# saltoricristiano/lidog

Measured on AMD Instinct MI355X. Metric: LiDAR scans/sec, MinkUNet34+BEV training step @120k pts, higher is better.
Workload: dtype f32

## Files before the change

### include/lidog_amd.h

```cpp
#ifndef LIDOG_AMD_H
#define LIDOG_AMD_H

#include <stdint.h>

#ifdef __cplusplus
extern "C" {
#endif

const char *lidog_last_error(void);
int lidog_abi_version(void);


int64_t lidog_hash_capacity(int64_t n);

int lidog_coords_insert(const int32_t *coords, int64_t n, uint64_t *keys, int32_t *vals, int64_t cap,
                        int32_t *first_row, int64_t *n_unique_dev, int32_t *err_flag, void *stream);
int lidog_coords_insert_info(const int32_t *coords, int64_t n, uint64_t *keys, int32_t *vals, int64_t cap,
                             int32_t *first_row, int64_t *info, int32_t *err_flag, void *stream);

int lidog_coords_compact(const int32_t *first_row, int64_t n, const uint64_t *keys, int32_t *vals, int64_t cap,
                         const int32_t *coords, int32_t *unique_rows, int32_t *inverse, int32_t *scan_ws,
                         void *stream);

int lidog_coords_stride(const int32_t *coords_in, int64_t n_in, int32_t new_stride, uint64_t *keys,
                        int32_t *vals, int64_t cap, int32_t *parent2child, int32_t *coords_out,
                        int64_t *n_out_dev, int32_t *ws, int32_t *err_flag, void *stream);

int64_t lidog_bitmap_words(int32_t nx, int32_t ny, int32_t nz, int32_t nb, int64_t max_bytes);
int lidog_bitmap_set(const int32_t *coords, int64_t n, int32_t x0, int32_t y0, int32_t z0, int32_t nx, int32_t ny,
                     int32_t nz, int32_t stride, int32_t nb, uint32_t *bits, int32_t *err_flag, void *stream);
int lidog_kernel_map_bits(const int32_t *coords_out, int64_t n_out, const uint64_t *in_keys, const int32_t *in_vals,
                          int64_t in_cap, const int32_t *offsets_host, int32_t K, const uint32_t *bits, int32_t x0,
                          int32_t y0, int32_t z0, int32_t nx, int32_t ny, int32_t nz, int32_t stride, int32_t nb,
                          int32_t *nbr, void *stream);
int lidog_kernel_map_subset(const int32_t *nbr_big, int64_t n, int32_t K_big, const int32_t *sel_host, int32_t K,
                            int32_t *nbr, void *stream);

int lidog_kernel_map(const int32_t *coords_out, int64_t n_out, const uint64_t *in_keys, const int32_t *in_vals,
                     int64_t in_cap, const int32_t *offsets_host, int32_t K, int32_t *nbr, void *stream);

int lidog_kernel_map_pairs(const int32_t *nbr, int64_t n_out, int64_t n_in, int32_t K, int64_t *k_off_dev,
                           int32_t *pair_in, int32_t *pair_out, int32_t *pos_out, int32_t *pos_in, int32_t *ws,
                           void *stream);
int lidog_kernel_map_rows(const int32_t *pos, int64_t n, int32_t K, int32_t mark_k, int32_t *row_ptr,
                          int32_t *row_list, int32_t *ws, void *stream);


int lidog_sconv_gemm(const float *A, const int32_t *gather, const float *B, const float *bias,
                     const int32_t *tile_k, const int32_t *tile_row0, const int32_t *tile_rows, int32_t n_tiles,
                     int32_t Cin, int32_t Cout, float *T, const int32_t *scatter, int64_t a_rows, void *stream);
int32_t lidog_sconv_gemm_units(int32_t multi, int32_t slots);
int lidog_sconv_gemm_addend(const float *A, const int32_t *gather, const float *B, const int32_t *tile_k,
                            const int32_t *tile_row0, const int32_t *tile_rows, int32_t n_tiles, int32_t Cin,
                            int32_t Cout, const float *addend, float *T, const int32_t *scatter, void *stream);

int lidog_sconv_reduce(const float *T, const int32_t *pos, int64_t n, int32_t K, int32_t C, const float *bias,
                       const float *addend ,
                       float *out, void *stream);

int64_t lidog_sconv_reduce_stats_ws(int64_t n, int32_t C);
int lidog_sconv_reduce_stats(const float *T, const int32_t *pos, int64_t n, int32_t K, int32_t C, const float *bias,
                             float *out, double *sums, double *partial_ws, double count, float eps, float momentum,
                             float *mean, float *invstd, float *running_mean, float *running_var, void *stream);
int lidog_sconv_reduce_rows(const float *T, const int32_t *row_ptr, const int32_t *row_list, int64_t n, int32_t C,
                            const float *bias, const float *addend, float *out, void *stream);
int lidog_sconv_reduce_rows_stats(const float *T, const int32_t *row_ptr, const int32_t *row_list, int64_t n,
                                  int32_t C, const float *bias, float *out, double *sums, double *partial_ws,
                                  double count, float eps, float momentum, float *mean, float *invstd,
// ... 287 lines not shown
```

### lidog_amd/_lib.py

```python
import ctypes
import os

import torch

_HERE = os.path.dirname(os.path.abspath(__file__))
SO_PATH = os.environ.get("LIDOG_SO") or os.path.join(_HERE, "_C", "liblidog_amd.so")

_i32, _i64, _p, _f, _d = ctypes.c_int32, ctypes.c_int64, ctypes.c_void_p, ctypes.c_float, ctypes.c_double

SIGNATURES = {
    "lidog_abi_version": [],
    "lidog_hash_capacity": [_i64],
    "lidog_coords_insert": [_p, _i64, _p, _p, _i64, _p, _p, _p, _p],
    "lidog_coords_insert_info": [_p, _i64, _p, _p, _i64, _p, _p, _p, _p],
    "lidog_coords_compact": [_p, _i64, _p, _p, _i64, _p, _p, _p, _p, _p],
    "lidog_coords_stride": [_p, _i64, _i32, _p, _p, _i64, _p, _p, _p, _p, _p, _p],
    "lidog_kernel_map": [_p, _i64, _p, _p, _i64, _p, _i32, _p, _p],
    "lidog_bitmap_words": [_i32, _i32, _i32, _i32, _i64],
    "lidog_bitmap_set": [_p, _i64, _i32, _i32, _i32, _i32, _i32, _i32, _i32, _i32, _p, _p, _p],
    "lidog_kernel_map_bits": [_p, _i64, _p, _p, _i64, _p, _i32, _p, _i32, _i32, _i32, _i32, _i32, _i32, _i32, _i32, _p, _p],
    "lidog_kernel_map_pairs": [_p, _i64, _i64, _i32, _p, _p, _p, _p, _p, _p, _p],
    "lidog_sconv_gemm_units": [_i32, _i32],
    "lidog_sconv_gemm": [_p, _p, _p, _p, _p, _p, _p, _i32, _i32, _i32, _p, _p, _i64, _p],
    "lidog_sconv_gemm_addend": [_p, _p, _p, _p, _p, _p, _i32, _i32, _i32, _p, _p, _p, _p],
    "lidog_sconv_reduce": [_p, _p, _i64, _i32, _i32, _p, _p, _p, _p],
    "lidog_sconv_reduce_stats_ws": [_i64, _i32],
    "lidog_sconv_reduce_stats": [_p, _p, _i64, _i32, _i32, _p, _p, _p, _p, _d, _f, _f, _p, _p, _p, _p, _p],
    "lidog_kernel_map_rows": [_p, _i64, _i32, _i32, _p, _p, _p, _p],
    "lidog_sconv_reduce_rows": [_p, _p, _p, _i64, _i32, _p, _p, _p, _p],
    "lidog_sconv_reduce_rows_bn": [_p, _p, _p, _i64, _i32, _p, _p, _p, _p, _p, _p, _i32, _p, _p],
    "lidog_sconv_reduce_rows_stats": [_p, _p, _p, _i64, _i32, _p, _p, _p, _p, _d, _f, _f, _p, _p, _p, _p, _p],
    "lidog_sconv_reduce_rows_bwdstats": [_p, _p, _p, _i64, _i32, _p, _p, _p, _p, _p, _p, _p, _p, _p, _p, _p, _d, _p, _p, _p],
    "lidog_bn_bwd_reduce_blocks": [_i64, _i32],
    "lidog_stats_max_blocks": [],
    "lidog_sconv_cin1": [_p, _p, _p, _p, _i64, _i32, _i32, _p, _p],
    "lidog_kernel_map_subset": [_p, _i64, _i32, _p, _i32, _p, _p],
    "lidog_kernel_map_sorted_ws": [_i64],
    "lidog_kernel_map_sorted": [_p, _i64, _i32, _p, _p, _p, _p, _p, _i64, _p],
    "lidog_sconv_os": [_p, _p, _i64, _i32, _p, _p, _p, _p, _i32, _p, _p, _i32, _i32, _p, _p],
    "lidog_sconv_os_stats_ws": [_i64, _i32],
    "lidog_sconv_os_bn": [_p, _p, _i64, _i32, _p, _p, _p, _p, _p, _i32, _i32, _p, _p, _p, _p, _p, _i32, _p, _p],
    "lidog_sconv_os_stats": [_p, _p, _i64, _i32, _p, _p, _p, _p, _p, _i32, _i32, _p, _p, _p, _d, _f, _f, _p, _p, _p, _p, _p],
    "lidog_sconv_wgrad": [_p, _p, _p, _p, _p, _i32, _p, _i32, _i32, _i32, _p, _p, _p],
    "lidog_sconv_gemm_in_bn": [_p, _p, _p, _p, _p, _p, _p, _i32, _i32, _i32, _p, _p, _p, _p, _p, _p, _i32, _i64, _p],
# ... 190 lines not shown
```

### lidog_amd/csrc/coords.hip

```cpp
#include <limits.h>
#include <stdarg.h>

#include "common.h"

static thread_local char g_err[512] = "";
void lidog_set_error(const char *fmt, ...) {
    va_list ap;
    va_start(ap, fmt);
    vsnprintf(g_err, sizeof(g_err), fmt, ap);
    va_end(ap);
}
extern "C" const char *lidog_last_error(void) { return g_err; }
extern "C" int lidog_abi_version(void) { return 8; }

extern "C" int64_t lidog_hash_capacity(int64_t n) {
    int64_t cap = 1024;
    while (cap < 2 * n) cap <<= 1;
    return cap;
}

__device__ __forceinline__ int block_excl_scan_256(int v, int *total) {
    __shared__ int wsum[4];
    const int lane = threadIdx.x & 63, w = threadIdx.x >> 6;
    int x = v;
// ... 51 lines not shown
    int v[4], s = 0;
#pragma unroll
    for (int j = 0; j < 4; ++j) {
        v[j] = (base + j < n) ? data[base + j] : 0;
        s += v[j];
    }
    int tot;
    int ex = block_excl_scan_256(s, &tot) + sums[blockIdx.x];
#pragma unroll
    for (int j = 0; j < 4; ++j) {
        if (base + j < n) data[base + j] = ex;
        ex += v[j];
    }
}

static int device_exclusive_scan(int32_t *data, int64_t n, int32_t *sums, hipStream_t st) {
    int64_t nb = cdiv64(n, 1024);
    if (nb == 0) return 0;
    scan_block_sums<<<dim3((unsigned)nb), 256, 0, st>>>(data, n, sums);
    scan_block_offsets<<<1, 256, 0, st>>>(sums, nb);
    scan_apply<<<dim3((unsigned)nb), 256, 0, st>>>(data, n, sums);
    LIDOG_LAUNCH_CHECK();
    return 0;
}

__device__ __forceinline__ int32_t table_insert_min(uint64_t *keys, int32_t *vals, uint64_t mask, uint64_t key,
                                                    int32_t row) {
    uint64_t slot = lidog_mix(key) & mask;
    for (;;) {
        unsigned long long prev = atomicCAS((unsigned long long *)&keys[slot], (unsigned long long)LIDOG_EMPTY_KEY,
                                            (unsigned long long)key);
        if (prev == LIDOG_EMPTY_KEY || prev == key) {
            atomicMin(&vals[slot], row);
            return (int32_t)slot;
        }
        slot = (slot + 1) & mask;
    }
}

__global__ __launch_bounds__(256) void k_insert(const int4 *__restrict__ coords, int64_t n, int32_t stride,
                                                uint64_t *keys, int32_t *vals, uint64_t mask,
                                                int32_t *__restrict__ slot_of, int32_t *err_flag) {
    int64_t i = (int64_t)blockIdx.x * 256 + threadIdx.x;
    if (i >= n) return;
    int4 c = coords[i];
    if (stride > 1) {
// ... 62 lines not shown
        for (int j = 0; j < 3; ++j) s_lo[w][j] = lo[j];
#pragma unroll
        for (int j = 0; j < 4; ++j) s_hi[w][j] = hi[j];
    }
    __syncthreads();
    if (threadIdx.x < 7) {
        const int j = threadIdx.x;
        if (j < 3) {
            int v = min(min(s_lo[0][j], s_lo[1][j]), min(s_lo[2][j], s_lo[3][j]));
            if (v != INT_MAX) atomicMin(&info[3 + j], (long long)v);
        } else {
            const int k = j - 3;
            int v = max(max(s_hi[0][k], s_hi[1][k]), max(s_hi[2][k], s_hi[3][k]));
            if (v != INT_MIN) atomicMax(&info[k < 3 ? 6 + k : 2], (long long)v);
        }
    }
}

extern "C" int lidog_coords_insert_info(const int32_t *coords, int64_t n, uint64_t *keys, int32_t *vals, int64_t cap,
                                        int32_t *first_row, int64_t *info, int32_t *err_flag, void *stream) {
    hipStream_t st = (hipStream_t)stream;
    LIDOG_REQUIRE(cap >= 2 * n && (cap & (cap - 1)) == 0, "coords_insert: cap must be a power of two >= 2n");
    LIDOG_REQUIRE(info != nullptr, "coords_insert_info: info buffer missing");
    LIDOG_CHECK_HIP(hipMemsetAsync(keys, 0xff, sizeof(uint64_t) * cap, st));
    LIDOG_CHECK_HIP(hipMemsetD32Async((hipDeviceptr_t)vals, 0x7fffffff, cap, st));
    k_info_init<<<1, 16, 0, st>>>((long long *)info);
    if (n == 0) return 0;
    unsigned nb = (unsigned)cdiv64(n, 256);
    k_insert_info<<<nb, 256, 0, st>>>((const int4 *)coords, n, keys, vals, (uint64_t)(cap - 1), first_row, err_flag,
                                      (long long *)info);
    k_first_row<<<nb, 256, 0, st>>>(first_row, n, vals, (unsigned long long *)info);
    LIDOG_LAUNCH_CHECK();
    return 0;
}

extern "C" int lidog_coords_insert(const int32_t *coords, int64_t n, uint64_t *keys, int32_t *vals, int64_t cap,
                                   int32_t *first_row, int64_t *n_unique_dev, int32_t *err_flag, void *stream) {
    hipStream_t st = (hipStream_t)stream;
    LIDOG_REQUIRE(cap >= 2 * n && (cap & (cap - 1)) == 0, "coords_insert: cap must be a power of two >= 2n");
    LIDOG_CHECK_HIP(hipMemsetAsync(keys, 0xff, sizeof(uint64_t) * cap, st));
    LIDOG_CHECK_HIP(hipMemsetD32Async((hipDeviceptr_t)vals, 0x7fffffff, cap, st));
    LIDOG_CHECK_HIP(hipMemsetAsync(n_unique_dev, 0, sizeof(int64_t), st));
    if (n == 0) return 0;
    unsigned nb = (unsigned)cdiv64(n, 256);
    k_insert<<<nb, 256, 0, st>>>((const int4 *)coords, n, 1, keys, vals, (uint64_t)(cap - 1), first_row, err_flag);
    k_first_row<<<nb, 256, 0, st>>>(first_row, n, vals, (unsigned long long *)n_unique_dev);
    LIDOG_LAUNCH_CHECK();
    return 0;
}

__global__ __launch_bounds__(256) void k_flag_first(const int32_t *__restrict__ first_row, int64_t n,
                                                    int32_t *__restrict__ flag) {
    int64_t i = (int64_t)blockIdx.x * 256 + threadIdx.x;
    if (i < n) flag[i] = (first_row[i] == (int)i);
}

__global__ __launch_bounds__(256) void k_compact_rows(const int32_t *__restrict__ first_row, int64_t n,
                                                      const int32_t *__restrict__ rank, const int4 *coords,
                                                      const uint64_t *keys, int32_t *vals, uint64_t mask,
                                                      int32_t *__restrict__ unique_rows,
                                                      int32_t *__restrict__ inverse) {
    int64_t i = (int64_t)blockIdx.x * 256 + threadIdx.x;
    if (i >= n) return;
    int f = first_row[i];
    int r = rank[f];
// ... 53 lines not shown
            return q * stride;
        };
        c.y = fl(c.y); c.z = fl(c.z); c.w = fl(c.w);
        coords_out[r] = c;
    }
    if (i == n - 1) *n_out_dev = (int64_t)rank[i] + (first ? 1 : 0);
}

__global__ __launch_bounds__(256) void k_stride_rewrite(int64_t n, const int32_t *__restrict__ slot_of,
                                                        int32_t *vals, const int32_t *__restrict__ rank,
                                                        const int32_t *__restrict__ parent2child) {
    int64_t i = (int64_t)blockIdx.x * 256 + threadIdx.x;
    if (i >= n) return;
    int s = slot_of[i];
    if (s >= 0 && parent2child[i] == rank[i]) vals[s] = rank[i];
}

extern "C" int lidog_coords_stride(const int32_t *coords_in, int64_t n_in, int32_t new_stride, uint64_t *keys,
                                   int32_t *vals, int64_t cap, int32_t *parent2child, int32_t *coords_out,
                                   int64_t *n_out_dev, int32_t *ws, int32_t *err_flag, void *stream) {
    hipStream_t st = (hipStream_t)stream;
    LIDOG_REQUIRE(cap >= 2 * n_in && (cap & (cap - 1)) == 0, "coords_stride: cap must be a power of two >= 2n");
    LIDOG_REQUIRE(n_in < 0x3fffffff, "coords_stride: too many rows");
    LIDOG_CHECK_HIP(hipMemsetAsync(keys, 0xff, sizeof(uint64_t) * cap, st));
    LIDOG_CHECK_HIP(hipMemsetD32Async((hipDeviceptr_t)vals, 0x7fffffff, cap, st));
    LIDOG_CHECK_HIP(hipMemsetAsync(n_out_dev, 0, sizeof(int64_t), st));
    if (n_in == 0) return 0;
    unsigned nb = (unsigned)cdiv64(n_in, 256);
    int32_t *slot_of = ws, *rank = ws + n_in, *sums = ws + 2 * n_in;
    k_insert<<<nb, 256, 0, st>>>((const int4 *)coords_in, n_in, new_stride, keys, vals, (uint64_t)(cap - 1), slot_of,
                                 err_flag);
    k_stride_flag<<<nb, 256, 0, st>>>(slot_of, n_in, vals, rank);
    if (device_exclusive_scan(rank, n_in, sums, st)) return 1;
    k_stride_emit<<<nb, 256, 0, st>>>((const int4 *)coords_in, n_in, new_stride, slot_of, vals, rank,
                                      (int4 *)coords_out, parent2child, n_out_dev);
    k_stride_rewrite<<<nb, 256, 0, st>>>(n_in, slot_of, vals, rank, parent2child);
    LIDOG_LAUNCH_CHECK();
    return 0;
}

struct KOffsets {
    int32_t d[125 * 3];
};

__global__ __launch_bounds__(256) void k_kernel_map(const int4 *__restrict__ coords_out, int64_t n_out,
                                                    const uint64_t *__restrict__ keys,
                                                    const int32_t *__restrict__ vals, uint64_t mask, KOffsets offs,
                                                    int32_t *__restrict__ nbr) {
    __shared__ int32_t s_off[125 * 3];
// ... 107 lines not shown
    int slabs = (K % 25 == 0) ? K / 25 : (K % 9 == 0) ? K / 9 : 1;
    dim3 grid((unsigned)cdiv64(n_out, 256), (unsigned)slabs);
    k_kernel_map_bits<<<grid, 256, 0, st>>>((const int4 *)coords_out, n_out, in_keys, in_vals, (uint64_t)(in_cap - 1),
                                            offs, K, bx, bits, nbr);
    LIDOG_LAUNCH_CHECK();
    return 0;
}

extern "C" int lidog_kernel_map(const int32_t *coords_out, int64_t n_out, const uint64_t *in_keys,
                                const int32_t *in_vals, int64_t in_cap, const int32_t *offsets_host, int32_t K,
                                int32_t *nbr, void *stream) {
    hipStream_t st = (hipStream_t)stream;
    LIDOG_REQUIRE(K >= 1 && K <= 125, "kernel_map: K=%d out of range [1,125]", K);
    if (n_out == 0) return 0;
    KOffsets offs;
    for (int i = 0; i < K * 3; ++i) offs.d[i] = offsets_host[i];
    dim3 grid((unsigned)cdiv64(n_out, 256), (unsigned)K);
    k_kernel_map<<<grid, 256, 0, st>>>((const int4 *)coords_out, n_out, in_keys, in_vals, (uint64_t)(in_cap - 1), offs,
                                       nbr);
    LIDOG_LAUNCH_CHECK();
    return 0;
}

struct KSubset {
    int32_t sel[27];
};

__global__ __launch_bounds__(256) void k_nbr_subset(const int4 *__restrict__ big, int64_t n, KSubset sel,
                                                    int4 *__restrict__ nbr) {
    const int64_t q = (int64_t)blockIdx.x * 256 + threadIdx.x;
    const int k = blockIdx.y;
    if (q * 4 >= n) return;
    nbr[(int64_t)k * (n / 4) + q] = big[(int64_t)sel.sel[k] * (n / 4) + q];
}

__global__ __launch_bounds__(256) void k_nbr_subset1(const int32_t *__restrict__ big, int64_t n, KSubset sel,
                                                     int32_t *__restrict__ nbr) {
    const int64_t r = (int64_t)blockIdx.x * 256 + threadIdx.x;
    const int k = blockIdx.y;
    if (r >= n) return;
    nbr[(int64_t)k * n + r] = big[(int64_t)sel.sel[k] * n + r];
}

extern "C" int lidog_kernel_map_subset(const int32_t *nbr_big, int64_t n, int32_t K_big, const int32_t *sel_host,
                                       int32_t K, int32_t *nbr, void *stream) {
    hipStream_t st = (hipStream_t)stream;
// ... 48 lines not shown
        if (threadIdx.x == 0) carry_s = carry + tot;
        __syncthreads();
    }
    if (threadIdx.x == 0) totals[k] = carry_s;
}

__global__ __launch_bounds__(128) void k_pairs_koff(const int32_t *__restrict__ totals, int K, int64_t *__restrict__ k_off) {
    __shared__ int64_t s[128];
    const int t = threadIdx.x;
    s[t] = t < K ? totals[t] : 0;
    __syncthreads();
    if (t == 0) {
        int64_t run = 0;
        for (int kk = 0; kk < K; ++kk) {
            k_off[kk] = run;
            run += s[kk];
        }
        k_off[K] = run;
    }
}

__global__ __launch_bounds__(256) void k_pairs_emit(const int32_t *__restrict__ nbr, int64_t n_out, int64_t n_in,
                                                    int nbp, const int32_t *__restrict__ cnt,
                                                    const int64_t *__restrict__ k_off, int32_t *__restrict__ pair_in,
                                                    int32_t *__restrict__ pair_out, int32_t *__restrict__ pos_out,
                                                    int32_t *__restrict__ pos_in) {
    const int k = blockIdx.y, b = blockIdx.x;
    const int lane = threadIdx.x & 63, w = threadIdx.x >> 6;
    __shared__ int wcnt[4][4];
    int nb_[4];
    unsigned long long masks[4];
#pragma unroll
    for (int j = 0; j < 4; ++j) {
        int64_t o = (int64_t)b * 1024 + j * 256 + threadIdx.x;
        nb_[j] = (o < n_out) ? nbr[(int64_t)k * n_out + o] : -1;
        masks[j] = __ballot(nb_[j] >= 0);
        if (lane == 0) wcnt[j][w] = __popcll(masks[j]);
    }
    __syncthreads();
    int64_t base = k_off[k] + cnt[(int64_t)k * nbp + b];
    int run = 0;
#pragma unroll
    for (int j = 0; j < 4; ++j) {
        int before = run;
        for (int ww = 0; ww < 4; ++ww) {
            if (ww < w) before += wcnt[j][ww];
            run += wcnt[j][ww];
        }
        int64_t o = (int64_t)b * 1024 + j * 256 + threadIdx.x;
        if (o < n_out) {
            int32_t p = -1;
            if (nb_[j] >= 0) {
                int rank = before + __popcll(masks[j] & ((1ull << lane) - 1ull));
                p = (int32_t)(base + rank);
                pair_in[p] = nb_[j];
                pair_out[p] = (int32_t)o;
                if (pos_in) pos_in[(int64_t)k * n_in + nb_[j]] = p;
            }
            if (pos_out) pos_out[(int64_t)k * n_out + o] = p;
        }
    }
}

extern "C" int lidog_kernel_map_pairs(const int32_t *nbr, int64_t n_out, int64_t n_in, int32_t K,
                                      int64_t *k_off_dev, int32_t *pair_in, int32_t *pair_out, int32_t *pos_out,
                                      int32_t *pos_in, int32_t *ws, void *stream) {
    hipStream_t st = (hipStream_t)stream;
    LIDOG_REQUIRE(K >= 1 && K <= 125, "kernel_map_pairs: K=%d out of range [1,125]", K);
    LIDOG_REQUIRE(n_out * (int64_t)K < 0x7fffffff, "kernel_map_pairs: pair positions overflow int32");
    if (pos_in) LIDOG_CHECK_HIP(hipMemsetAsync(pos_in, 0xff, sizeof(int32_t) * n_in * K, st));
    if (n_out == 0) {
        LIDOG_CHECK_HIP(hipMemsetAsync(k_off_dev, 0, sizeof(int64_t) * (K + 1), st));
        return 0;
    }
    int nbp = (int)cdiv64(n_out, 1024);
    int32_t *cnt = ws, *totals = ws + (int64_t)nbp * K;
    dim3 grid((unsigned)nbp, (unsigned)K);
    k_pairs_count<<<grid, 256, 0, st>>>(nbr, n_out, nbp, cnt);
    k_pairs_scan<<<(unsigned)K, 256, 0, st>>>(cnt, nbp, totals);
    k_pairs_koff<<<1, 128, 0, st>>>(totals, K, k_off_dev);
    k_pairs_emit<<<grid, 256, 0, st>>>(nbr, n_out, n_in, nbp, cnt, k_off_dev, pair_in, pair_out, pos_out, pos_in);
    LIDOG_LAUNCH_CHECK();
    return 0;
}

__global__ __launch_bounds__(256) void k_rows_count(const int32_t *__restrict__ pos, int64_t n, int K,
                                                    int32_t *__restrict__ row_ptr) {
    const int64_t o = (int64_t)blockIdx.x * 256 + threadIdx.x;
    if (o > n) return;
    int c = 0;
    if (o < n)
        for (int k = 0; k < K; ++k) c += pos[(int64_t)k * n + o] >= 0;
    row_ptr[o] = c;
}

__global__ __launch_bounds__(256) void k_rows_fill(const int32_t *__restrict__ pos, int64_t n, int K, int mark_k,
                                                   const int32_t *__restrict__ row_ptr,
                                                   int32_t *__restrict__ row_list) {
    const int64_t o = (int64_t)blockIdx.x * 256 + threadIdx.x;
    if (o >= n) return;
    int p = row_ptr[o];
    for (int k = 0; k < K; ++k) {
        const int v = pos[(int64_t)k * n + o];
        if (v >= 0) row_list[p++] = k == mark_k ? -1 : v;
    }
}

extern "C" int lidog_kernel_map_rows(const int32_t *pos, int64_t n, int32_t K, int32_t mark_k, int32_t *row_ptr,
                                     int32_t *row_list, int32_t *ws, void *stream) {
    hipStream_t st = (hipStream_t)stream;
    LIDOG_REQUIRE(n >= 0 && K >= 1 && n < ((int64_t)1 << 31) - 2, "kernel_map_rows: bad sizes");
    k_rows_count<<<(unsigned)cdiv64(n + 1, 256), 256, 0, st>>>(pos, n, K, row_ptr);
    if (device_exclusive_scan(row_ptr, n + 1, ws, st)) return 1;
    if (n) k_rows_fill<<<(unsigned)cdiv64(n, 256), 256, 0, st>>>(pos, n, K, mark_k, row_ptr, row_list);
    LIDOG_LAUNCH_CHECK();
    return 0;
}
```

### lidog_amd/me.py

```python
import ctypes
import math
import os
import sys
import types

import numpy as np
import torch
import torch.nn as nn

from . import _lib
from ._lib import call, call_on, ptr

TILE_ROWS = 128


def kernel_offsets(kernel_size, tensor_stride, dilation=1):
    k = int(kernel_size)
    if k % 2 == 1:
        r = [(-(k // 2) + i) * tensor_stride * dilation for i in range(k)]
    else:
        r = [i * tensor_stride * dilation for i in range(k)]
    return np.array([(x, y, z) for z in r for y in r for x in r], dtype=np.int32)


# ... 30 lines not shown
            out.append(dev[off:off + a.size].view(a.shape))
            off += a.size
        return dev, out


class _CoordMap:
    __slots__ = ("coords", "keys", "vals", "cap", "n", "bits", "box", "segs")

    def __init__(self, coords, keys, vals, cap):
        self.coords, self.keys, self.vals, self.cap, self.n = coords, keys, vals, cap, coords.shape[0]
        self.bits = self.box = None
        self.segs = None


class KernelMap:

    def __init__(self, K, n_in, n_out, k_off, k_off_host, pair_in, pair_out, pos_out, pos_in, nbr, tiles=None):
        self.K, self.n_in, self.n_out = K, n_in, n_out
        self.k_off, self.k_off_host = k_off, k_off_host
        self.P = int(k_off_host[-1])
        self.pair_in, self.pair_out, self._pos_out, self._pos_in, self.nbr = pair_in, pair_out, pos_out, pos_in, nbr
        self.tiles, self.n_tiles = tiles if tiles is not None else _tiles(k_off_host, pair_in.device)
        self._rows = {}

    def _pos_table(self, side):
        name = "_pos_" + side
        t = getattr(self, name)
        if t is None:
            n = self.n_out if side == "out" else self.n_in
            rows = (self.pair_out if side == "out" else self.pair_in).long()
            dev = rows.device
            t = torch.full((self.K, n), -1, dtype=torch.int32, device=dev)
            counts = torch.tensor(np.diff(np.asarray(self.k_off_host, dtype=np.int64)), device=dev)
            ks = torch.repeat_interleave(torch.arange(self.K, device=dev), counts)
            t[ks, rows] = torch.arange(self.P, dtype=torch.int32, device=dev)
            setattr(self, name, t)
        return t

    pos_out = property(lambda self: self._pos_table("out"))
    pos_in = property(lambda self: self._pos_table("in"))

    def sorted(self):
        if "_sorted" not in self.__dict__:
            self._sorted = None
            ok = _SCONV_OS and self.K == 27 and self.n_in == self.n_out and self.nbr is not None and self.n_out > 0
            if ok and (_SCONV_OS == 2 or (self.P <= _SCONV_OS_DENSITY * self.n_out and
                                          self.n_out >= 128 * _SCONV_OS_MIN_TILES)):
                n, dev = self.n_out, self.nbr.device
                pad = (n + 127) // 128 * 128
                perm = torch.empty(pad, dtype=torch.int32, device=dev)
                wmask = torch.empty(pad // 32, dtype=torch.int32, device=dev)
                order = torch.empty(pad // 128, dtype=torch.int32, device=dev)
                ws = torch.empty(_lib.load().lidog_kernel_map_sorted_ws(n), dtype=torch.uint8, device=dev)
                call("lidog_kernel_map_sorted", ptr(self.nbr), n, self.K, ptr(self.k_off), ptr(perm), ptr(wmask),
                     ptr(order), ptr(ws), ws.numel())
                self._sorted = (perm, wmask, order)
        return self._sorted

    def rows(self, side):
        key = side
        if key not in self._rows:
            pos, n = (self.pos_out, self.n_out) if side == "out" else (self.pos_in, self.n_in)
            dev = pos.device
            row_ptr = torch.empty(n + 1, dtype=torch.int32, device=dev)
            row_list = torch.empty(max(self.P, 1), dtype=torch.int32, device=dev)
            ws = torch.empty((n + 1 + 1023) // 1024 + 1, dtype=torch.int32, device=dev)
            call("lidog_kernel_map_rows", ptr(pos), n, self.K, -1, ptr(row_ptr),
                 ptr(row_list), ptr(ws))
            self._rows[key] = (row_ptr, row_list)
        return self._rows[key]


class _IdentityMap:

    def __init__(self, n, device, tiles=None):
        self.K, self.n_in, self.n_out, self.P = 1, n, n, n
        self.k_off_host = [0, n]
        self.k_off = torch.tensor([0, n], dtype=torch.int64, device=device)
        self.rows = torch.arange(n, dtype=torch.int32, device=device)
        self.tiles, self.n_tiles = tiles if tiles is not None else _tiles(self.k_off_host, device)


_SIDE_STREAMS = {}
_SCONV_OS = int(os.environ.get("LIDOG_SCONV_OS", "1"))
_SCONV_OS_DENSITY = float(os.environ.get("LIDOG_SCONV_OS_DENSITY", "6.0"))
_SCONV_OS_MIN_TILES = int(os.environ.get("LIDOG_SCONV_OS_MIN_TILES", "1500"))
_OS_HINT = {}


def _side_stream(device):
    key = torch.device(device).index if torch.device(device).index is not None else torch.cuda.current_device()
# ... 195 lines not shown
        if stats[0] != n:
            m = int(stats[0])
            uniq_full = torch.empty(n, dtype=torch.int32, device=self.device)
            inv = torch.empty(n, dtype=torch.int32, device=self.device)
            ws = torch.empty(n + 2048, dtype=torch.int32, device=self.device)
            call("lidog_coords_compact", ptr(first), n, ptr(keys), ptr(vals), cap, ptr(coords), ptr(uniq_full),
                 ptr(inv), ptr(ws))
            uniq = uniq_full[:m]
            coords = coords[uniq.long()].contiguous()
            self._own(uniq_full, inv, coords)
        self.maps[1] = _CoordMap(coords, keys, vals, cap)
        return uniq, inv

    def stride(self, s_in, s_out):
        if s_out in self.maps:
            return self.maps[s_out]
        src = self.maps[s_in]
        n = src.n
        cap = _lib.load().lidog_hash_capacity(n)
        keys = self._own(torch.empty(cap, dtype=torch.int64, device=self.device))
        vals = self._own(torch.empty(cap, dtype=torch.int32, device=self.device))
        p2c = torch.empty(n, dtype=torch.int32, device=self.device)
        out = self._own(torch.empty((n, 4), dtype=torch.int32, device=self.device))
        n_out = torch.zeros(1, dtype=torch.int64, device=self.device)
        ws = torch.empty(2 * n + 2048, dtype=torch.int32, device=self.device)
        call("lidog_coords_stride", ptr(src.coords), n, int(s_out), ptr(keys), ptr(vals), cap, ptr(p2c), ptr(out),
             ptr(n_out), ptr(ws), ptr(self.err))
        m = int(n_out.item())
        self.maps[s_out] = _CoordMap(out[:m], keys, vals, cap)
        return self.maps[s_out]

    def _bitmap(self, s):
        cmap = self.maps[s]
        if cmap.box is not None:
            return cmap.bits, cmap.box
        cmap.box = ()
        if not _BITMAPS or getattr(self, "bounds", None) is None or cmap.n < _BITMAP_MIN_ROWS:
            return None, ()
        lo, hi = self.bounds
        x0 = [(int(v) // s) * s for v in lo]
        nn = [(int(h) // s) * s // s - a // s + 1 for h, a in zip(hi, x0)]
        words = _lib.load().lidog_bitmap_words(nn[0], nn[1], nn[2], self.batch_size, _BITMAP_MAX_BYTES)
        if words < 0:
            return None, ()
        bits = self._own(torch.zeros(words, dtype=torch.int32, device=self.device))
        box = (x0[0], x0[1], x0[2], nn[0], nn[1], nn[2], s, self.batch_size)
        call("lidog_bitmap_set", ptr(cmap.coords), cmap.n, *box, ptr(bits), ptr(self.err))
        cmap.bits, cmap.box = bits, box
        return bits, box

    def kernel_map(self, s_in, s_out, kernel_size, dilation=1):
        key = (s_in, s_out, kernel_size, dilation)
        if key in self.kmaps:
            return self.kmaps[key]
        if s_out != s_in:
            self.stride(s_in, s_out)
        pd = self._kernel_map_launch(key)
        k_off_host = torch.cat([pd[3], self.err.long()]).tolist()
        if k_off_host.pop() != 0:
            self._check()
        self.kmaps[key] = self._kernel_map_finish(pd, k_off_host, None, key)
        return self.kmaps[key]

    def _kernel_map_launch(self, key):
        s_in, s_out, kernel_size, dilation = key
        cin = self.maps[s_in]
        cout = cin if s_out == s_in else self.maps[s_out]
        offs = kernel_offsets(kernel_size, s_in, dilation)
        K = offs.shape[0]
        n_in, n_out = cin.n, cout.n
        nbr = torch.empty((K, n_out), dtype=torch.int32, device=self.device)
        big = self._nbr_tables.get((s_in, s_out, 5, dilation)) if (_SUBSET_MAPS and kernel_size == 3 and s_in == s_out) else None
        bits, box = (None, None) if big is not None else self._bitmap(s_in)
        if big is not None:
            call("lidog_kernel_map_subset", ptr(big), n_out, 125, _SUBSET_3_OF_5.ctypes.data, K, ptr(nbr))
        elif bits is not None:
            call("lidog_kernel_map_bits", ptr(cout.coords), n_out, ptr(cin.keys), ptr(cin.vals), cin.cap,
                 offs.ctypes.data, K, ptr(bits), *box, ptr(nbr))
        else:
            call("lidog_kernel_map", ptr(cout.coords), n_out, ptr(cin.keys), ptr(cin.vals), cin.cap,
                 offs.ctypes.data, K, ptr(nbr))
        k_off = torch.empty(K + 1, dtype=torch.int64, device=self.device)
        pair_in = torch.empty(n_out * K, dtype=torch.int32, device=self.device)
        pair_out = torch.empty(n_out * K, dtype=torch.int32, device=self.device)
        by_row = K <= 27 and not (K == 27 and s_in == s_out and _OS_HINT.get(key, False))
        pos_out = torch.empty((K, n_out), dtype=torch.int32, device=self.device) if by_row else None
        pos_in = torch.empty((K, n_in), dtype=torch.int32, device=self.device) if by_row else None
        nbp = (n_out + 1023) // 1024
        ws = torch.empty((nbp + 1) * K + K + 2, dtype=torch.int32, device=self.device)
        call("lidog_kernel_map_pairs", ptr(nbr), n_out, n_in, K, ptr(k_off), ptr(pair_in), ptr(pair_out),
             ptr(pos_out), ptr(pos_in), ptr(ws))
        self._own(*[t for t in (nbr, k_off, pair_in, pair_out, pos_out, pos_in) if t is not None])
        self._nbr_tables[key] = nbr
        return (K, n_in, n_out, k_off, pair_in, pair_out, pos_out, pos_in, nbr)

    def _kernel_map_finish(self, pd, k_off_host, tiles, key=None):
        K, n_in, n_out, k_off, pair_in, pair_out, pos_out, pos_in, nbr = pd
        P = int(k_off_host[-1])
        m = KernelMap(K, n_in, n_out, k_off, k_off_host, pair_in[:P], pair_out[:P], pos_out, pos_in, nbr, tiles)
        if K == 27:
            srt = m.sorted()
            if key is not None:
                _OS_HINT[key] = srt is not None
            if srt is not None:
                self._own(*srt)
            else:
                self._own(*m.rows("out"), *m.rows("in"))
        elif K == 8:
            self._own(*m.rows("out"))
        return m

    def segments(self, key):
        cmap = self.maps[key]
        if cmap.segs is None:
            n, B = cmap.n, int(self.batch_size or 0)
            perm = torch.empty(n, dtype=torch.int32, device=self.device)
            seg_off = torch.empty(B + 1, dtype=torch.int32, device=self.device)
            bid = torch.empty(n, dtype=torch.int32, device=self.device)
            nbytes = _lib.load().lidog_in_segments_ws(n)
            ws = torch.empty(nbytes, dtype=torch.uint8, device=self.device)
            call("lidog_in_segments", ptr(cmap.coords), n, B, ptr(perm), ptr(seg_off), ptr(bid), ptr(ws), nbytes)
            cmap.segs = self._own(perm, seg_off, bid) + (B,)
# ... 130 lines not shown
    ref = getattr(param, "_flat_ref", None)
    if ref is None or param.grad is not None:
        return None
    buf, off, owner = ref
    if param._flat_taken == owner.generation:
        lane = wgrad_lane(buf.device) if buf.is_cuda else None
        if lane is not None:
            torch.cuda.current_stream(buf.device).wait_stream(lane.stream)
        return None
    param._flat_taken = owner.generation
    return buf[off:off + param.numel()].view(shape)


def _gemm(A, gather, B, bias, m, Cin, Cout, out, scatter, tiles=None):
    desc, n_tiles = (tiles[0], tiles[1]) if tiles is not None else (m.tiles, m.n_tiles)
    call("lidog_sconv_gemm", ptr(A), ptr(gather), ptr(B), ptr(bias), ptr(desc[0]), ptr(desc[1]), ptr(desc[2]),
         n_tiles, Cin, Cout, ptr(out), ptr(scatter), A.shape[0])


_SUBSET_3_OF_5 = np.array([(dz + 2) * 25 + (dy + 2) * 5 + (dx + 2) for dz in (-1, 0, 1) for dy in (-1, 0, 1)
                           for dx in (-1, 0, 1)], dtype=np.int32)
_SUBSET_MAPS = os.environ.get("LIDOG_MAP_SUBSET", "1") != "0"
_BITMAPS = os.environ.get("LIDOG_MAP_BITMAPS", "1") != "0"
_BITMAP_MAX_BYTES = int(os.environ.get("LIDOG_MAP_BITMAP_MAX_MB", "1024")) << 20
_BITMAP_MIN_ROWS = 40000


_WGRAD_TARGET_BLOCKS = int(os.environ.get("LIDOG_WGRAD_BLOCKS", "2048"))
_WGRAD_WIDE_BLOCKS = _WGRAD_TARGET_BLOCKS // 2


_WGRAD_FIT = int(os.environ.get("LIDOG_WGRAD_FIT", "-1"))
_wgrad_slots_cache = {}


def _wgrad_slots(Cin, Cout):
    key = (Cin, Cout)
    if key not in _wgrad_slots_cache:
        _wgrad_slots_cache[key] = int(_lib.load().lidog_sconv_wgrad_slots(Cin, Cout, 0))
    return _wgrad_slots_cache[key]


def _wgrad_chunk(k_off_host, Cin, Cout):
    P = int(k_off_host[-1]) - int(k_off_host[0])

    def tile(c):
# ... 838 lines not shown
```

Baseline: 84.86.

## Build kernel maps with fused counting and symmetric mirroring, fusing table init fills

Adds a counted kernel-map builder that queries only half the offsets for same-stride odd kernels and writes the mirrored entries by symmetry. It also accumulates the per-block pair counts and per-row counts inside the lookup, so the separate count pass, the k_off kernel and the row-pointer counting can be skipped later. Hash-table initialisation memsets are replaced by a single vectorised fill kernel, and pos_in shares the -1 filled buffer with nbr. The cost is more atomics in the lookup kernel and more complex bookkeeping. Correctness relies on the offset symmetry and the assumption that input and output coordinate sets are the same.

```diff
diff --git a/include/lidog_amd.h b/include/lidog_amd.h
--- a/include/lidog_amd.h
+++ b/include/lidog_amd.h
@@ -44,6 +44,18 @@
                            void *stream);
 int lidog_kernel_map_rows(const int32_t *pos, int64_t n, int32_t K, int32_t mark_k, int32_t *row_ptr,
                           int32_t *row_list, int32_t *ws, void *stream);
+
+int lidog_kernel_map_counted(const int32_t *coords_out, int64_t n_out, const uint64_t *in_keys, const int32_t *in_vals,
+                             int64_t in_cap, const int32_t *offsets_host, int32_t K, int32_t symmetric,
+                             const uint32_t *bits, int32_t x0, int32_t y0, int32_t z0, int32_t nx, int32_t ny,
+                             int32_t nz, int32_t stride, int32_t nb, int32_t *nbr, int32_t *cnt, int32_t *row_cnt,
+                             int32_t *zero, int64_t zero_ints, int32_t *ones, int64_t ones_ints, int32_t slab,
+                             void *stream);
+int lidog_kernel_map_pairs_counted(const int32_t *nbr, int64_t n_out, int64_t n_in, int32_t K, int64_t *k_off_dev,
+                                   int32_t *pair_in, int32_t *pair_out, int32_t *pos_out, int32_t *pos_in, int32_t *ws,
+                                   int32_t pos_in_filled, void *stream);
+int lidog_kernel_map_rows_counted(const int32_t *pos, int64_t n, int32_t K, int32_t mark_k, int32_t *row_ptr,
+                                  int32_t scanned, int32_t *row_list, int32_t *ws, void *stream);
 
 
 int lidog_sconv_gemm(const float *A, const int32_t *gather, const float *B, const float *bias,
diff --git a/lidog_amd/_lib.py b/lidog_amd/_lib.py
--- a/lidog_amd/_lib.py
+++ b/lidog_amd/_lib.py
@@ -20,6 +20,10 @@
     "lidog_bitmap_set": [_p, _i64, _i32, _i32, _i32, _i32, _i32, _i32, _i32, _i32, _p, _p, _p],
     "lidog_kernel_map_bits": [_p, _i64, _p, _p, _i64, _p, _i32, _p, _i32, _i32, _i32, _i32, _i32, _i32, _i32, _i32, _p, _p],
     "lidog_kernel_map_pairs": [_p, _i64, _i64, _i32, _p, _p, _p, _p, _p, _p, _p],
+    "lidog_kernel_map_counted": [_p, _i64, _p, _p, _i64, _p, _i32, _i32, _p, _i32, _i32, _i32, _i32, _i32, _i32, _i32,
+                                 _i32, _p, _p, _p, _p, _i64, _p, _i64, _i32, _p],
+    "lidog_kernel_map_pairs_counted": [_p, _i64, _i64, _i32, _p, _p, _p, _p, _p, _p, _i32, _p],
+    "lidog_kernel_map_rows_counted": [_p, _i64, _i32, _i32, _p, _i32, _p, _p, _p],
     "lidog_sconv_gemm_units": [_i32, _i32],
     "lidog_sconv_gemm": [_p, _p, _p, _p, _p, _p, _p, _i32, _i32, _i32, _p, _p, _i64, _p],
     "lidog_sconv_gemm_addend": [_p, _p, _p, _p, _p, _p, _i32, _i32, _i32, _p, _p, _p, _p],
diff --git a/lidog_amd/csrc/coords.hip b/lidog_amd/csrc/coords.hip
--- a/lidog_amd/csrc/coords.hip
+++ b/lidog_amd/csrc/coords.hip
@@ -97,6 +97,47 @@
     scan_apply<<<dim3((unsigned)nb), 256, 0, st>>>(data, n, sums);
     LIDOG_LAUNCH_CHECK();
     return 0;
+}
+
+struct FillRegions {
+    int32_t *p[3];
+    int64_t n[3];
+    int32_t v[3];
+};
+
+__device__ __forceinline__ void fill_region(int32_t *__restrict__ p, int64_t n, int32_t v, int64_t tid, int64_t nt) {
+    int64_t head = (4 - (int64_t)(((uintptr_t)p >> 2) & 3)) & 3;
+    if (head > n) head = n;
+    if (tid < head) p[tid] = v;
+    int4 *q = (int4 *)(p + head);
+    const int64_t nq = (n - head) / 4;
+    for (int64_t i = tid; i < nq; i += nt) q[i] = make_int4(v, v, v, v);
+    const int64_t tail0 = head + nq * 4;
+    if (tid < n - tail0) p[tail0 + tid] = v;
+}
+
+__global__ __launch_bounds__(256) void k_fill_regions(FillRegions r) {
+    const int64_t tid = (int64_t)blockIdx.x * 256 + threadIdx.x, nt = (int64_t)gridDim.x * 256;
+#pragma unroll
+    for (int i = 0; i < 3; ++i)
+        if (r.p[i] && r.n[i] > 0) fill_region(r.p[i], r.n[i], r.v[i], tid, nt);
+}
+
+static int launch_fill(FillRegions r, hipStream_t st) {
+    int64_t most = 0;
+    for (int i = 0; i < 3; ++i)
+        if (r.p[i] && r.n[i] > most) most = r.n[i];
+    if (most == 0) return 0;
+    int64_t blocks = cdiv64(most / 4 + 1, 256);
+    if (blocks > 2048) blocks = 2048;
+    k_fill_regions<<<(unsigned)blocks, 256, 0, st>>>(r);
+    LIDOG_LAUNCH_CHECK();
+    return 0;
+}
+
+static int launch_table_init(uint64_t *keys, int32_t *vals, int64_t cap, int64_t *counter, hipStream_t st) {
+    FillRegions r{{(int32_t *)keys, vals, (int32_t *)counter}, {2 * cap, cap, counter ? 2 : 0}, {-1, 0x7fffffff, 0}};
+    return launch_fill(r, st);
 }
 
 __device__ __forceinline__ int32_t table_insert_min(uint64_t *keys, int32_t *vals, uint64_t mask, uint64_t key,
@@ -205,8 +246,7 @@
     hipStream_t st = (hipStream_t)stream;
     LIDOG_REQUIRE(cap >= 2 * n && (cap & (cap - 1)) == 0, "coords_insert: cap must be a power of two >= 2n");
     LIDOG_REQUIRE(info != nullptr, "coords_insert_info: info buffer missing");
-    LIDOG_CHECK_HIP(hipMemsetAsync(keys, 0xff, sizeof(uint64_t) * cap, st));
-    LIDOG_CHECK_HIP(hipMemsetD32Async((hipDeviceptr_t)vals, 0x7fffffff, cap, st));
+    if (launch_table_init(keys, vals, cap, nullptr, st)) return 1;
     k_info_init<<<1, 16, 0, st>>>((long long *)info);
     if (n == 0) return 0;
     unsigned nb = (unsigned)cdiv64(n, 256);
@@ -221,9 +261,7 @@
                                    int32_t *first_row, int64_t *n_unique_dev, int32_t *err_flag, void *stream) {
     hipStream_t st = (hipStream_t)stream;
     LIDOG_REQUIRE(cap >= 2 * n && (cap & (cap - 1)) == 0, "coords_insert: cap must be a power of two >= 2n");
-    LIDOG_CHECK_HIP(hipMemsetAsync(keys, 0xff, sizeof(uint64_t) * cap, st));
-    LIDOG_CHECK_HIP(hipMemsetD32Async((hipDeviceptr_t)vals, 0x7fffffff, cap, st));
-    LIDOG_CHECK_HIP(hipMemsetAsync(n_unique_dev, 0, sizeof(int64_t), st));
+    if (launch_table_init(keys, vals, cap, n_unique_dev, st)) return 1;
     if (n == 0) return 0;
     unsigned nb = (unsigned)cdiv64(n, 256);
     k_insert<<<nb, 256, 0, st>>>((const int4 *)coords, n, 1, keys, vals, (uint64_t)(cap - 1), first_row, err_flag);
@@ -323,9 +361,7 @@
     hipStream_t st = (hipStream_t)stream;
     LIDOG_REQUIRE(cap >= 2 * n_in && (cap & (cap - 1)) == 0, "coords_stride: cap must be a power of two >= 2n");
     LIDOG_REQUIRE(n_in < 0x3fffffff, "coords_stride: too many rows");
-    LIDOG_CHECK_HIP(hipMemsetAsync(keys, 0xff, sizeof(uint64_t) * cap, st));
-    LIDOG_CHECK_HIP(hipMemsetD32Async((hipDeviceptr_t)vals, 0x7fffffff, cap, st));
-    LIDOG_CHECK_HIP(hipMemsetAsync(n_out_dev, 0, sizeof(int64_t), st));
+    if (launch_table_init(keys, vals, cap, n_out_dev, st)) return 1;
     if (n_in == 0) return 0;
     unsigned nb = (unsigned)cdiv64(n_in, 256);
     int32_t *slot_of = ws, *rank = ws + n_in, *sums = ws + 2 * n_in;
@@ -479,6 +515,133 @@
     return 0;
 }
 
+template <bool SYM, bool BITS>
+__global__ __launch_bounds__(256) void k_kernel_map_cnt(const int4 *__restrict__ coords_out, int64_t n_out,
+                                                        const uint64_t *__restrict__ keys,
+                                                        const int32_t *__restrict__ vals, uint64_t mask, KOffsets offs,
+                                                        int K, int k_hi, int per, BitBox bx,
+                                                        const uint32_t *__restrict__ bits, int32_t *__restrict__ nbr,
+                                                        int nbp, int32_t *__restrict__ cnt,
+                                                        int32_t *__restrict__ row_cnt) {
+    __shared__ int32_t s_off[125 * 3];
+    for (int t = threadIdx.x; t < K * 3; t += 256) s_off[t] = offs.d[t];
+    __syncthreads();
+    const int64_t o = (int64_t)blockIdx.x * 256 + threadIdx.x;
+    const bool valid = o < n_out;
+    const int lane = threadIdx.x & 63;
+    const int b = (int)(((int64_t)blockIdx.x * 256 + (threadIdx.x & ~63)) >> 10);
+    const int4 c = valid ? coords_out[o] : make_int4(0, 0, 0, 0);
+    const int k_begin = (int)blockIdx.y * per, k_end = k_begin + per < k_hi ? k_begin + per : k_hi;
+    int own = 0;
+    for (int k0 = k_begin; k0 < k_end; k0 += 5) {
+        int64_t idx[5];
+        uint32_t word[5];
+        if (BITS) {
+#pragma unroll
+            for (int j = 0; j < 5; ++j) {
+                const int k = k0 + j < k_end ? k0 + j : k_end - 1;
+                idx[j] = valid ? bit_index(bx, c.x, c.y + s_off[3 * k], c.z + s_off[3 * k + 1], c.w + s_off[3 * k + 2]) : -1;
+                word[j] = bits[idx[j] >= 0 ? idx[j] >> 5 : 0];
+            }
+        }
+#pragma unroll
+        for (int j = 0; j < 5; ++j) {
+            const int k = k0 + j;
+            if (k >= k_end) break;
+            int32_t row = -1;
+            if (valid && (!BITS || (idx[j] >= 0 && ((word[j] >> (idx[j] & 31)) & 1u)))) {
+                int bad = 0;
+                uint64_t key = lidog_pack(c.x, c.y + s_off[3 * k], c.z + s_off[3 * k + 1], c.w + s_off[3 * k + 2], &bad);
+                row = bad ? -1 : lidog_find(keys, vals, mask, key);
+            }
+            if (valid) nbr[(int64_t)k * n_out + o] = row;
+            const bool hit = row >= 0;
+            const unsigned long long m = __ballot(hit);
+            if (lane == 0 && m) atomicAdd(&cnt[(int64_t)k * nbp + b], __popcll(m));
+            own += hit;
+            if (SYM) {
+                const int km = K - 1 - k;
+                const bool mir = hit && row < n_out;
+                if (mir) {
+                    nbr[(int64_t)km * n_out + row] = (int32_t)o;
+                    if (row_cnt) atomicAdd(&row_cnt[row], 1);
+                }
+                const int jb = mir ? row >> 10 : -1;
+                unsigned long long pend = __ballot(mir);
+                while (pend) {
+                    const int leader = __ffsll((long long)pend) - 1;
+                    const int bl = __shfl(jb, leader);
+                    const unsigned long long same = __ballot(mir && jb == bl);
+                    if (lane == leader) atomicAdd(&cnt[(int64_t)km * nbp + bl], __popcll(same));
+                    pend &= ~same;
+                }
+            }
+        }
+    }
+    if (SYM && blockIdx.y == 0) {
+        if (valid) nbr[(int64_t)(K / 2) * n_out + o] = (int32_t)o;
+        const unsigned long long m = __ballot(valid);
+        if (lane == 0 && m) atomicAdd(&cnt[(int64_t)(K / 2) * nbp + b], __popcll(m));
+        own += valid;
+    }
+    if (row_cnt && valid && own) atomicAdd(&row_cnt[o], own);
+}
+
+extern "C" int lidog_kernel_map_counted(const int32_t *coords_out, int64_t n_out, const uint64_t *in_keys,
+                                        const int32_t *in_vals, int64_t in_cap, const int32_t *offsets_host, int32_t K,
+                                        int32_t symmetric, const uint32_t *bits, int32_t x0, int32_t y0, int32_t z0,
+                                        int32_t nx, int32_t ny, int32_t nz, int32_t stride, int32_t nb, int32_t *nbr,
+                                        int32_t *cnt, int32_t *row_cnt, int32_t *zero, int64_t zero_ints, int32_t *ones,
+                                        int64_t ones_ints, int32_t slab, void *stream) {
+    hipStream_t st = (hipStream_t)stream;
+    LIDOG_REQUIRE(K >= 1 && K <= 125, "kernel_map_counted: K=%d out of range [1,125]", K);
+    LIDOG_REQUIRE(n_out >= 0 && n_out < 0x7fffffff && cnt != nullptr && slab >= 0, "kernel_map_counted: bad arguments");
+    if (bits) LIDOG_REQUIRE(stride >= 1 && nx > 0 && ny > 0 && nz > 0 && nb > 0, "kernel_map_counted: bad box");
+    const int nbp = (int)cdiv64(n_out, 1024);
+    if (symmetric) {
+        LIDOG_REQUIRE(K % 2 == 1, "kernel_map_counted: a symmetric map needs an odd kernel, K=%d", K);
+        for (int k = 0; k < K; ++k)
+            for (int a = 0; a < 3; ++a)
+                LIDOG_REQUIRE(offsets_host[3 * (K - 1 - k) + a] == -offsets_host[3 * k + a],
+                              "kernel_map_counted: offset %d is not the negative of offset %d", K - 1 - k, k);
+    }
+    if (zero) {
+        LIDOG_REQUIRE(cnt >= zero && cnt + (int64_t)K * nbp <= zero + zero_ints &&
+                      (!row_cnt || (row_cnt >= zero && row_cnt + n_out + 1 <= zero + zero_ints)),
+                      "kernel_map_counted: the counters lie outside the zero-filled region");
+    }
+    if (ones) {
+        LIDOG_REQUIRE(!symmetric || (ones <= nbr + (int64_t)(K / 2 + 1) * n_out && nbr + (int64_t)K * n_out <= ones + ones_ints),
+                      "kernel_map_counted: the upper half of the table lies outside the -1-filled region");
+    }
+    {
+        FillRegions r{{zero, ones, nullptr}, {zero ? zero_ints : 0, ones ? ones_ints : 0, 0}, {0, -1, 0}};
+        if (launch_fill(r, st)) return 1;
+    }
+    if (n_out == 0) return 0;
+    KOffsets offs;
+    for (int i = 0; i < K * 3; ++i) offs.d[i] = offsets_host[i];
+    BitBox bx{x0, y0, z0, nx, ny, nz, stride > 0 ? stride : 1, nb};
+    const int k_hi = symmetric ? K / 2 : K;
+    int per = slab ? slab : symmetric ? (K == 125 ? 15 : 5) : (K % 25 == 0) ? 25 : (K % 9 == 0) ? 9 : K;
+    if (per > k_hi) per = k_hi;
+    if (per < 1) per = 1;
+    const int slabs = k_hi > 0 ? (k_hi + per - 1) / per : 1;
+    dim3 grid((unsigned)cdiv64(n_out, 256), (unsigned)slabs);
+    const int4 *co = (const int4 *)coords_out;
+    const uint64_t mask = (uint64_t)(in_cap - 1);
+#define LIDOG_MAP_CNT(S, B) \
+    k_kernel_map_cnt<S, B><<<grid, 256, 0, st>>>(co, n_out, in_keys, in_vals, mask, offs, K, k_hi, per, bx, bits, nbr, nbp, cnt, row_cnt)
+    if (symmetric) {
+        if (bits) LIDOG_MAP_CNT(true, true); else LIDOG_MAP_CNT(true, false);
+    } else {
+        if (bits) LIDOG_MAP_CNT(false, true); else LIDOG_MAP_CNT(false, false);
+    }
+#undef LIDOG_MAP_CNT
+    LIDOG_LAUNCH_CHECK();
+    return 0;
+}
+
 struct KSubset {
     int32_t sel[27];
 };
@@ -573,12 +736,38 @@
 
 __global__ __launch_bounds__(256) void k_pairs_emit(const int32_t *__restrict__ nbr, int64_t n_out, int64_t n_in,
                                                     int nbp, const int32_t *__restrict__ cnt,
-                                                    const int64_t *__restrict__ k_off, int32_t *__restrict__ pair_in,
+                                                    int64_t *__restrict__ k_off, int32_t *__restrict__ pair_in,
                                                     int32_t *__restrict__ pair_out, int32_t *__restrict__ pos_out,
-                                                    int32_t *__restrict__ pos_in) {
+                                                    int32_t *__restrict__ pos_in,
+                                                    const int32_t *__restrict__ totals) {
     const int k = blockIdx.y, b = blockIdx.x;
     const int lane = threadIdx.x & 63, w = threadIdx.x >> 6;
     __shared__ int wcnt[4][4];
+    __shared__ long long s_koff[2];
+    if (totals) {
+        if (w == 0) {
+            const int K = gridDim.y;
+            long long below = 0, all = 0;
+            for (int t = lane; t < K; t += 64) {
+                const int v = totals[t];
+                all += v;
+                if (t < k) below += v;
+            }
+#pragma unroll
+            for (int d = 32; d >= 1; d >>= 1) {
+                below += __shfl_xor(below, d);
+                all += __shfl_xor(all, d);
+            }
+            if (lane == 0) {
+                s_koff[0] = below;
+                s_koff[1] = all;
+                if (b == 0) {
+                    k_off[k] = below;
+                    if (k == K - 1) k_off[K] = all;
+                }
+            }
+        }
+    }
     int nb_[4];
     unsigned long long masks[4];
 #pragma unroll
@@ -589,7 +778,7 @@
         if (lane == 0) wcnt[j][w] = __popcll(masks[j]);
     }
     __syncthreads();
-    int64_t base = k_off[k] + cnt[(int64_t)k * nbp + b];
+    int64_t base = (totals ? (int64_t)s_koff[0] : k_off[k]) + cnt[(int64_t)k * nbp + b];
     int run = 0;
 #pragma unroll
     for (int j = 0; j < 4; ++j) {
@@ -630,7 +819,29 @@
     k_pairs_count<<<grid, 256, 0, st>>>(nbr, n_out, nbp, cnt);
     k_pairs_scan<<<(unsigned)K, 256, 0, st>>>(cnt, nbp, totals);
     k_pairs_koff<<<1, 128, 0, st>>>(totals, K, k_off_dev);
-    k_pairs_emit<<<grid, 256, 0, st>>>(nbr, n_out, n_in, nbp, cnt, k_off_dev, pair_in, pair_out, pos_out, pos_in);
+    k_pairs_emit<<<grid, 256, 0, st>>>(nbr, n_out, n_in, nbp, cnt, k_off_dev, pair_in, pair_out, pos_out, pos_in,
+                                       nullptr);
+    LIDOG_LAUNCH_CHECK();
+    return 0;
+}
+
+extern "C" int lidog_kernel_map_pairs_counted(const int32_t *nbr, int64_t n_out, int64_t n_in, int32_t K,
+                                              int64_t *k_off_dev, int32_t *pair_in, int32_t *pair_out,
+                                              int32_t *pos_out, int32_t *pos_in, int32_t *ws, int32_t pos_in_filled,
+                                              void *stream) {
+    hipStream_t st = (hipStream_t)stream;
+    LIDOG_REQUIRE(K >= 1 && K <= 125, "kernel_map_pairs: K=%d out of range [1,125]", K);
+    LIDOG_REQUIRE(n_out * (int64_t)K < 0x7fffffff, "kernel_map_pairs: pair positions overflow int32");
+    if (pos_in && !pos_in_filled) LIDOG_CHECK_HIP(hipMemsetAsync(pos_in, 0xff, sizeof(int32_t) * n_in * K, st));
+    if (n_out == 0) {
+        LIDOG_CHECK_HIP(hipMemsetAsync(k_off_dev, 0, sizeof(int64_t) * (K + 1), st));
+        return 0;
+    }
+    int nbp = (int)cdiv64(n_out, 1024);
+    int32_t *cnt = ws, *totals = ws + (int64_t)nbp * K;
+    dim3 grid((unsigned)nbp, (unsigned)K);
+    k_pairs_scan<<<(unsigned)K, 256, 0, st>>>(cnt, nbp, totals);
+    k_pairs_emit<<<grid, 256, 0, st>>>(nbr, n_out, n_in, nbp, cnt, k_off_dev, pair_in, pair_out, pos_out, pos_in, totals);
     LIDOG_LAUNCH_CHECK();
     return 0;
 }
@@ -667,3 +878,39 @@
     LIDOG_LAUNCH_CHECK();
     return 0;
 }
+
+__global__ __launch_bounds__(256) void scan_apply_raw(int32_t *__restrict__ data, int64_t n,
+                                                      const int32_t *__restrict__ sums) {
+    int below = 0;
+    for (int64_t i = threadIdx.x; i < (int64_t)blockIdx.x; i += 256) below += sums[i];
+    int carry;
+    block_excl_scan_256(below, &carry);
+    int64_t base = (int64_t)blockIdx.x * 1024 + threadIdx.x * 4;
+    int v[4], s = 0;
+#pragma unroll
+    for (int j = 0; j < 4; ++j) {
+        v[j] = (base + j < n) ? data[base + j] : 0;
+        s += v[j];
+    }
+    int tot;
+    int ex = block_excl_scan_256(s, &tot) + carry;
+#pragma unroll
+    for (int j = 0; j < 4; ++j) {
+        if (base + j < n) data[base + j] = ex;
+        ex += v[j];
+    }
+}
+
+extern "C" int lidog_kernel_map_rows_counted(const int32_t *pos, int64_t n, int32_t K, int32_t mark_k, int32_t *row_ptr,
+                                             int32_t scanned, int32_t *row_list, int32_t *ws, void *stream) {
+    hipStream_t st = (hipStream_t)stream;
+    LIDOG_REQUIRE(n >= 0 && K >= 1 && n < ((int64_t)1 << 31) - 2, "kernel_map_rows: bad sizes");
+    if (!scanned) {
+        const int64_t nb = cdiv64(n + 1, 1024);
+        scan_block_sums<<<dim3((unsigned)nb), 256, 0, st>>>(row_ptr, n + 1, ws);
+        scan_apply_raw<<<dim3((unsigned)nb), 256, 0, st>>>(row_ptr, n + 1, ws);
+    }
+    if (n) k_rows_fill<<<(unsigned)cdiv64(n, 256), 256, 0, st>>>(pos, n, K, mark_k, row_ptr, row_list);
+    LIDOG_LAUNCH_CHECK();
+    return 0;
+}
diff --git a/lidog_amd/me.py b/lidog_amd/me.py
--- a/lidog_amd/me.py
+++ b/lidog_amd/me.py
@@ -76,6 +76,7 @@
         self.pair_in, self.pair_out, self._pos_out, self._pos_in, self.nbr = pair_in, pair_out, pos_out, pos_in, nbr
         self.tiles, self.n_tiles = tiles if tiles is not None else _tiles(k_off_host, pair_in.device)
         self._rows = {}
+        self._row_counts = None
 
     def _pos_table(self, side):
         name = "_pos_" + side
@@ -116,11 +117,19 @@
         if key not in self._rows:
             pos, n = (self.pos_out, self.n_out) if side == "out" else (self.pos_in, self.n_in)
             dev = pos.device
-            row_ptr = torch.empty(n + 1, dtype=torch.int32, device=dev)
             row_list = torch.empty(max(self.P, 1), dtype=torch.int32, device=dev)
             ws = torch.empty((n + 1 + 1023) // 1024 + 1, dtype=torch.int32, device=dev)
-            call("lidog_kernel_map_rows", ptr(pos), n, self.K, -1, ptr(row_ptr),
-                 ptr(row_list), ptr(ws))
+            counts, sym = self._row_counts if self._row_counts is not None else (None, False)
+            if counts is not None and (side == "out" or sym):
+                if side == "in" and "out" not in self._rows:
+                    self.rows("out")
+                row_ptr = counts
+                call("lidog_kernel_map_rows_counted", ptr(pos), n, self.K, -1, ptr(row_ptr), int(side == "in"),
+                     ptr(row_list), ptr(ws))
+            else:
+                row_ptr = torch.empty(n + 1, dtype=torch.int32, device=dev)
+                call("lidog_kernel_map_rows", ptr(pos), n, self.K, -1, ptr(row_ptr),
+                     ptr(row_list), ptr(ws))
             self._rows[key] = (row_ptr, row_list)
         return self._rows[key]
 
@@ -362,7 +371,7 @@
         vals = self._own(torch.empty(cap, dtype=torch.int32, device=self.device))
         p2c = torch.empty(n, dtype=torch.int32, device=self.device)
         out = self._own(torch.empty((n, 4), dtype=torch.int32, device=self.device))
-        n_out = torch.zeros(1, dtype=torch.int64, device=self.device)
+        n_out = torch.empty(1, dtype=torch.int64, device=self.device)
         ws = torch.empty(2 * n + 2048, dtype=torch.int32, device=self.device)
         call("lidog_coords_stride", ptr(src.coords), n, int(s_out), ptr(keys), ptr(vals), cap, ptr(p2c), ptr(out),
              ptr(n_out), ptr(ws), ptr(self.err))
@@ -409,9 +418,11 @@
         offs = kernel_offsets(kernel_size, s_in, dilation)
         K = offs.shape[0]
         n_in, n_out = cin.n, cout.n
-        nbr = torch.empty((K, n_out), dtype=torch.int32, device=self.device)
         big = self._nbr_tables.get((s_in, s_out, 5, dilation)) if (_SUBSET_MAPS and kernel_size == 3 and s_in == s_out) else None
         bits, box = (None, None) if big is not None else self._bitmap(s_in)
+        if big is None and _MAP_SYM:
+            return self._kernel_map_launch_counted(key, cin, cout, offs, bits, box)
+        nbr = torch.empty((K, n_out), dtype=torch.int32, device=self.device)
         if big is not None:
             call("lidog_kernel_map_subset", ptr(big), n_out, 125, _SUBSET_3_OF_5.ctypes.data, K, ptr(nbr))
         elif bits is not None:
@@ -432,12 +443,39 @@
              ptr(pos_out), ptr(pos_in), ptr(ws))
         self._own(*[t for t in (nbr, k_off, pair_in, pair_out, pos_out, pos_in) if t is not None])
         self._nbr_tables[key] = nbr
-        return (K, n_in, n_out, k_off, pair_in, pair_out, pos_out, pos_in, nbr)
+        return (K, n_in, n_out, k_off, pair_in, pair_out, pos_out, pos_in, nbr, None)
+
+    def _kernel_map_launch_counted(self, key, cin, cout, offs, bits, box):
+        s_in, s_out, kernel_size, dilation = key
+        K, n_in, n_out, dev = offs.shape[0], cin.n, cout.n, self.device
+        sym = _MAP_SYM == 1 and s_in == s_out and kernel_size % 2 == 1
+        by_row = K <= 27 and not (K == 27 and s_in == s_out and _OS_HINT.get(key, False))
+        tab = torch.empty((K, n_out) if not by_row else (K * (n_out + n_in),), dtype=torch.int32, device=dev)
+        nbr = tab if not by_row else tab[:K * n_out].view(K, n_out)
+        pos_in = tab[K * n_out:].view(K, n_in) if by_row else None
+        pos_out = torch.empty((K, n_out), dtype=torch.int32, device=dev) if by_row else None
+        ones = tab.view(-1)[((K // 2 + 1) * n_out if sym else K * n_out):]
+        nbp = (n_out + 1023) // 1024
+        ws_len = ((nbp + 1) * K + K + 2 + 3) // 4 * 4
+        zero = torch.empty(ws_len + (n_out + 1 if by_row else 0), dtype=torch.int32, device=dev)
+        ws, row_cnt = zero[:ws_len], (zero[ws_len:] if by_row else None)
+        call("lidog_kernel_map_counted", ptr(cout.coords), n_out, ptr(cin.keys), ptr(cin.vals), cin.cap,
+             offs.ctypes.data, K, int(sym), ptr(bits), *(box if bits is not None else (0,) * 8), ptr(nbr), ptr(ws),
+             ptr(row_cnt), ptr(zero), zero.numel(), ptr(ones) if ones.numel() else None, ones.numel(), 0)
+        k_off = torch.empty(K + 1, dtype=torch.int64, device=dev)
+        pair_in = torch.empty(n_out * K, dtype=torch.int32, device=dev)
+        pair_out = torch.empty(n_out * K, dtype=torch.int32, device=dev)
+        call("lidog_kernel_map_pairs_counted", ptr(nbr), n_out, n_in, K, ptr(k_off), ptr(pair_in), ptr(pair_out),
+             ptr(pos_out), ptr(pos_in), ptr(ws), 1)
+        self._own(tab, zero, k_off, pair_in, pair_out, *([pos_out] if by_row else []))
+        self._nbr_tables[key] = nbr
+        return (K, n_in, n_out, k_off, pair_in, pair_out, pos_out, pos_in, nbr, (row_cnt, sym) if by_row else None)
 
     def _kernel_map_finish(self, pd, k_off_host, tiles, key=None):
-        K, n_in, n_out, k_off, pair_in, pair_out, pos_out, pos_in, nbr = pd
+        K, n_in, n_out, k_off, pair_in, pair_out, pos_out, pos_in, nbr, counts = pd
         P = int(k_off_host[-1])
         m = KernelMap(K, n_in, n_out, k_off, k_off_host, pair_in[:P], pair_out[:P], pos_out, pos_in, nbr, tiles)
+        m._row_counts = counts
         if K == 27:
             srt = m.sorted()
             if key is not None:
@@ -614,6 +652,7 @@
                            for dx in (-1, 0, 1)], dtype=np.int32)
 _SUBSET_MAPS = os.environ.get("LIDOG_MAP_SUBSET", "1") != "0"
 _BITMAPS = os.environ.get("LIDOG_MAP_BITMAPS", "1") != "0"
+_MAP_SYM = int(os.environ.get("LIDOG_MAP_SYM", "1"))
 _BITMAP_MAX_BYTES = int(os.environ.get("LIDOG_MAP_BITMAP_MAX_MB", "1024")) << 20
 _BITMAP_MIN_ROWS = 40000
 
```

After: 85.32 (median of 6 runs). No clear change (+0.5%).
